# IGLICT/NeRFFaceEditing

Hardware: NVIDIA B200
Metric: rendered rays/sec (48+48 samples) (higher is better)
Workload: dtype f32 (gather, compositing) + bf16x3 split tensor-core MLP with f32 accumulate

## Files before the change

### nerffaceediting_b200/csrc/nfe_field_pipe2.cu

```cuda
#include <type_traits>

#include "nfe_field_launch.cuh"
#include "nfe_mlp_tc.cuh"

namespace nfe {

using namespace tcmlp;

namespace p2 {

constexpr int EPI_GROUPS = 2;
constexpr int MMA_WARP = 8;
constexpr int TAP_WARP0 = 9, TAP_WARPS = 3;
static_assert(TAP_WARPS >= 1 && TAP_WARPS <= 3, "tap warps are warps 9-11");
constexpr int GATHER_WARP0 = 12, GATHER_WARPS = 8;
constexpr int THREADS = (GATHER_WARP0 + GATHER_WARPS) * 32;
constexpr int PASSES_PER_TILE = TILE_M / 4;
constexpr int PER_LONG = (PASSES_PER_TILE + GATHER_WARPS - 1) / GATHER_WARPS;
constexpr int LONG_WARPS = PASSES_PER_TILE - (PER_LONG - 1) * GATHER_WARPS;
static_assert(LONG_WARPS >= 1 && LONG_WARPS <= GATHER_WARPS && PER_LONG >= 2, "bad gather split");
constexpr int TAP_BUFS = 3;
constexpr int GROUP_COLS = 192;
constexpr int P2_TMEM_COLS = 512;
constexpr int COL_D2 = 128;
constexpr int REC_STAGE_STRIDE = 208;

constexpr int REGS_LAUNCH = 65536 / THREADS / 8 * 8;
constexpr int REGS_EPI = 104, REGS_MISC = 64, REGS_GATHER = 104;
static_assert(REGS_EPI > REGS_LAUNCH && REGS_GATHER > REGS_LAUNCH && REGS_MISC < REGS_LAUNCH,
              "the epilogue and gather groups only grow, the MMA / tap group only shrinks");
static_assert(8 * (REGS_EPI - REGS_LAUNCH) + GATHER_WARPS * (REGS_GATHER - REGS_LAUNCH) <= 4 * (REGS_LAUNCH - REGS_MISC),
              "setmaxnreg.inc would wait forever");
static_assert((2 * REGS_EPI + REGS_MISC + (GATHER_WARPS / 4) * REGS_GATHER) * 32 <= 16384, "register file of a sub-partition");

constexpr float LOG2E = 1.4426950408889634f;
constexpr float LN2 = 0.6931471805599453f;

template <int KIND, bool SPLIT>
struct Smem {
    using T = TcTraits<KIND>;
    static constexpr int PARTS = SPLIT ? 2 : 1;
    static constexpr int NETS = T::HAS_B ? 2 : 1;
    alignas(128) unsigned char a1[2][T::SETS][PARTS][A1_BYTES];
    alignas(128) unsigned char b1[NETS][PARTS][B1_BYTES];
    alignas(128) unsigned char b2a[PARTS][(T::N_A / 8) * B2_SBO];
    alignas(128) unsigned char b2b[PARTS][(T::N_B / 8) * B2_SBO];
    alignas(16) uint4 taps[TAP_BUFS][TILE_M][7];
    alignas(16) float aff[TAP_BUFS][2][2][96];
    int aff_item[TAP_BUFS];
    alignas(16) unsigned char recbuf[EPI_GROUPS][TILE_M][REC_STAGE_STRIDE];
    float bias1[NETS][HIDDEN];
    float bias2a[T::N_A];
    float bias2b[T::N_B];
    alignas(8) uint64_t full[2], empty[2];
    uint64_t taps_full[TAP_BUFS], taps_empty[TAP_BUFS];
    uint64_t d1_full[2], a2a_full[2], a2b_full[2], d2a_full[2], d2b_full[2], d2_free[2];
    uint32_t tmem_base;
};

__device__ __forceinline__ void tmem_st8(uint32_t taddr, const uint32_t* r)
{
    asm volatile("tcgen05.st.sync.aligned.32x32b.x8.b32 [%0], {%1, %2, %3, %4, %5, %6, %7, %8};\n"
                 :: "r"(taddr), "r"(r[0]), "r"(r[1]), "r"(r[2]), "r"(r[3]), "r"(r[4]), "r"(r[5]), "r"(r[6]), "r"(r[7]) : "memory");
}

template <int KIND, bool SPLIT>
__device__ void load_params(Smem<KIND, SPLIT>& s, const nfe_mlp& net_a, const nfe_mlp& net_b)
{
    using T = TcTraits<KIND>;
    constexpr int PARTS = SPLIT ? 2 : 1;
    load_weights<PARTS>(s.b1[0][0], B1_BYTES, net_a.w1, net_a.wgain1, HIDDEN, HIDDEN, FEAT, B1_LBO, B1_SBO);
    load_weights<PARTS>(s.b2a[0], sizeof(s.b2a[0]), net_a.w2, net_a.wgain2 * LN2, T::OUT_A, T::N_A, HIDDEN, B2_LBO, B2_SBO);
    for (int i = threadIdx.x; i < HIDDEN; i += blockDim.x) s.bias1[0][i] = folded_bias(net_a.b1, net_a.bgain1, i) * LOG2E;
    for (int i = threadIdx.x; i < T::N_A; i += blockDim.x) s.bias2a[i] = i < T::OUT_A ? folded_bias(net_a.b2, net_a.bgain2, i) : 0.0f;
    if constexpr (T::HAS_B) {
        load_weights<PARTS>(s.b1[1][0], B1_BYTES, net_b.w1, net_b.wgain1, HIDDEN, HIDDEN, FEAT, B1_LBO, B1_SBO);
        load_weights<PARTS>(s.b2b[0], sizeof(s.b2b[0]), net_b.w2, net_b.wgain2 * LN2, T::OUT_B, T::N_B, HIDDEN, B2_LBO, B2_SBO);
        for (int i = threadIdx.x; i < HIDDEN; i += blockDim.x) s.bias1[1][i] = folded_bias(net_b.b1, net_b.bgain1, i) * LOG2E;
        for (int i = threadIdx.x; i < T::N_B; i += blockDim.x) s.bias2b[i] = i < T::OUT_B ? folded_bias(net_b.b2, net_b.bgain2, i) : 0.0f;
    }
}

__device__ __forceinline__ float2 rgb_activation2(float2 x)
{
    const float2 n = fmul2(x, make_float2(-LOG2E, -LOG2E));
    float e0, e1, r0, r1;
    asm("ex2.approx.ftz.f32 %0, %1;" : "=f"(e0) : "f"(n.x));
    asm("ex2.approx.ftz.f32 %0, %1;" : "=f"(e1) : "f"(n.y));
    const float2 d = fadd2(make_float2(e0, e1), make_float2(1.0f, 1.0f));
    asm("rcp.approx.ftz.f32 %0, %1;" : "=f"(r0) : "f"(d.x));
    asm("rcp.approx.ftz.f32 %0, %1;" : "=f"(r1) : "f"(d.y));
    return ffma2(make_float2(r0, r1), make_float2(1.002f, 1.002f), make_float2(-0.001f, -0.001f));
}

template <bool SPLIT>
__device__ __forceinline__ void hidden_in_place(uint32_t taddr, const float* bias1_log2)
{
    const float2 k2 = make_float2(LOG2E, LOG2E), one2 = make_float2(1.0f, 1.0f), neg2 = make_float2(-1.0f, -1.0f);
#pragma unroll 1
    for (int q = 0; q < HIDDEN / 16; ++q) {
        float v[16];
        tc::tmem_ld16(taddr + q * 16, v);
        tc::tmem_ld_wait();
        uint32_t hi[8], lo[8];
#pragma unroll
        for (int i = 0; i < 4; ++i) {
            const float4 b4 = *reinterpret_cast<const float4*>(bias1_log2 + q * 16 + 4 * i);
#pragma unroll
            for (int j = 0; j < 2; ++j) {
                const float2 t = ffma2(make_float2(v[4 * i + 2 * j], v[4 * i + 2 * j + 1]), k2, j ? make_float2(b4.z, b4.w) : make_float2(b4.x, b4.y));
                float e0, e1, l0, l1;
                asm("ex2.approx.ftz.f32 %0, %1;" : "=f"(e0) : "f"(-fabsf(t.x)));
                asm("ex2.approx.ftz.f32 %0, %1;" : "=f"(e1) : "f"(-fabsf(t.y)));
                const float2 s1 = fadd2(make_float2(e0, e1), one2);
                asm("lg2.approx.ftz.f32 %0, %1;" : "=f"(l0) : "f"(s1.x));
                asm("lg2.approx.ftz.f32 %0, %1;" : "=f"(l1) : "f"(s1.y));
                const float2 hh = fadd2(make_float2(fmaxf(t.x, 0.0f), fmaxf(t.y, 0.0f)), make_float2(l0, l1));
                const __nv_bfloat162 p = __floats2bfloat162_rn(hh.x, hh.y);
                hi[2 * i + j] = *reinterpret_cast<const uint32_t*>(&p);
                if (SPLIT) {
                    const float2 d = ffma2(__bfloat1622float2(p), neg2, hh);
                    const __nv_bfloat162 r = __floats2bfloat162_rn(d.x, d.y);
                    lo[2 * i + j] = *reinterpret_cast<const uint32_t*>(&r);
                }
            }
        }
        tmem_st8(taddr + q * 16, hi);
        if (SPLIT) tmem_st8(taddr + q * 16 + 8, lo);
    }
    tc::tmem_st_wait();
}

template <bool SPLIT>
__device__ __forceinline__ void issue_layer2(bool leader, uint32_t tmem_d, uint32_t tmem_h, const unsigned char* b_hi, const unsigned char* b_lo, uint32_t idesc)
{
    uint32_t acc = 0;
    const uint64_t db0 = tc::make_desc(0, B2_LBO, B2_SBO);
    const uint32_t bh = tc::smem_u32(b_hi) >> 4, bl = tc::smem_u32(b_lo) >> 4;
    constexpr int TERMS = SPLIT ? 3 : 1;
#pragma unroll
    for (int t = 0; t < TERMS; ++t) {
        const uint32_t part = (t == 1) ? 8u : 0u;
        const uint32_t b = (t == 2) ? bl : bh;
#pragma unroll
        for (int ks = 0; ks < HIDDEN / 16; ++ks) {
            if (leader) tc::mma_bf16_ts(tmem_d, tmem_h + ks * 16 + part, db0 + (b + ks * ((2 * B2_LBO) >> 4)), idesc, acc);
            acc = 1;
        }
    }
}

struct SampleRef { int64_t idx; int item; int64_t ray; };

__device__ __forceinline__ SampleRef sample_of(const FieldArgs& a, int64_t L, bool small)
{
    SampleRef r;
    r.idx = L;
    if (small) {
        r.item = (int)((uint32_t)L / (uint32_t)a.m);
        r.ray = (int64_t)((uint32_t)L / (uint32_t)a.s_per_ray);
    } else {
        r.item = (int)(L / a.m);
        r.ray = L / a.s_per_ray;
    }
    return r;
}

__device__ __forceinline__ float4 ldg_tap(const float4* lane_base, uint32_t off4, bool streaming)
{
    uint64_t addr;
    asm("mad.wide.u32 %0, %1, 16, %2;" : "=l"(addr) : "r"(off4), "l"(lane_base));
    if (streaming) return __ldcg(reinterpret_cast<const float4*>(addr));
    return __ldg(reinterpret_cast<const float4*>(addr));
}

#ifdef NFE_PIPE_PROFILE
__device__ unsigned long long g_p2_prof[4][16];
#define P2_WAIT(slot, bar, par) do { const long long t0_ = clock64(); tc::mbar_wait(bar, par); prof_[slot] += clock64() - t0_; } while (0)
#else
#define P2_WAIT(slot, bar, par) tc::mbar_wait(bar, par)
#endif

template <int REGS>
__device__ __forceinline__ void regs_inc() { asm volatile("setmaxnreg.inc.sync.aligned.u32 %0;" :: "n"(REGS)); }
template <int REGS>
__device__ __forceinline__ void regs_dec() { asm volatile("setmaxnreg.dec.sync.aligned.u32 %0;" :: "n"(REGS)); }

template <int KIND, bool SPLIT>
__global__ void __launch_bounds__(THREADS, 1) field_pipe2_kernel(FieldArgs a, nfe_mlp net_a, nfe_mlp net_b)
{
    using T = TcTraits<KIND>;
    constexpr int P = SPLIT ? 1 : 0;
    extern __shared__ __align__(128) unsigned char smem_raw[];
    Smem<KIND, SPLIT>& s = *reinterpret_cast<Smem<KIND, SPLIT>*>(smem_raw);
    const int warp = __shfl_sync(0xffffffffu, (int)(threadIdx.x >> 5), 0), lane = threadIdx.x & 31;

    if (warp == MMA_WARP) tc::tmem_alloc(&s.tmem_base, P2_TMEM_COLS);
    if (threadIdx.x == 0) {
        for (int i = 0; i < 2; ++i) {
            tc::mbar_init(&s.full[i], GATHER_WARPS);
            tc::mbar_init(&s.empty[i], 1);
            tc::mbar_init(&s.d1_full[i], 1);
            tc::mbar_init(&s.a2a_full[i], 4);
            tc::mbar_init(&s.a2b_full[i], 4);
            tc::mbar_init(&s.d2a_full[i], 1);
            tc::mbar_init(&s.d2b_full[i], 1);
            tc::mbar_init(&s.d2_free[i], 4);
        }
        for (int i = 0; i < TAP_BUFS; ++i) {
            tc::mbar_init(&s.taps_full[i], TAP_WARPS);
            tc::mbar_init(&s.taps_empty[i], GATHER_WARPS);
        }
        tc::mbar_fence_init();
    }
    load_params(s, net_a, net_b);
    tc::fence_async_smem();
    tc::fence_before_sync();
    __syncthreads();
    tc::fence_after_sync();
    const uint32_t tmem = s.tmem_base;
    const int64_t n_tiles = (a.total + TILE_M - 1) / TILE_M;
    const int64_t G = gridDim.x;
    const int n_my = (int)((n_tiles - blockIdx.x + G - 1) / G);
    const bool skip_b = a.sigma_only && KIND == NFE_DEC_DISENTANGLED;
    const bool has_b = T::HAS_B && !skip_b;
#ifdef NFE_PIPE_PROFILE
    long long prof_[16] = {};
    const long long prof_t0_ = clock64();
#endif

    if (warp >= GATHER_WARP0) {
        const int gw = warp - GATHER_WARP0;
        const int g = lane >> 3, c4 = lane & 7;
        const float4* set_a = reinterpret_cast<const float4*>(a.set_norm) + c4;
        const float4* set_b = reinterpret_cast<const float4*>(a.set_denorm) + c4;
        const bool affine = T::SETS == 2 && a.affine_scale != nullptr;
        const bool rolling = T::SETS == 1 || affine || skip_b;
        const float4* set_r = T::SETS == 2 ? set_a : set_b;
        const int n_pass = gw < LONG_WARPS ? PER_LONG : PER_LONG - 1;
        const int pass0 = gw < LONG_WARPS ? gw * PER_LONG : LONG_WARPS * PER_LONG + (gw - LONG_WARPS) * (PER_LONG - 1);
        const int row0 = 4 * pass0 + g;
        regs_inc<REGS_GATHER>();

        float4 va[12];
        if (n_my > 0) {
            P2_WAIT(0, &s.taps_full[0], 0);
            if (rolling) {
                const uint4* src = s.taps[0][row0];
#pragma unroll
                for (int q = 0; q < 3; ++q) {
                    const uint4 o4 = src[q];
                    va[4 * q] = ldg_tap(set_r, o4.x, q != 0); va[4 * q + 1] = ldg_tap(set_r, o4.y, q != 0);
                    va[4 * q + 2] = ldg_tap(set_r, o4.z, q != 0); va[4 * q + 3] = ldg_tap(set_r, o4.w, q != 0);
                }
            }
        }
        int tb = 0, tb_next = 1;
        for (int it = 0; it < n_my; ++it) {
            const int st = it & 1;
            const bool has_next = it + 1 < n_my;
            P2_WAIT(1, &s.empty[st], ((it >> 1) & 1) ^ 1);
            if (rolling) {
                auto tile_body = [&](auto np_tag) {
                    constexpr int NP = decltype(np_tag)::value;
                    const uint4* tap_row = s.taps[tb][row0];
#pragma unroll 1
                    for (int p = 0; p < NP; ++p) {
                        const int row = row0 + 4 * p;
                        const uint4* cur = tap_row + 4 * p * 7;
                        const bool more = p + 1 < NP;
                        const bool fetch = more || has_next;
                        if (!more && has_next) P2_WAIT(0, &s.taps_full[tb_next], ((it + 1) / TAP_BUFS) & 1);
                        const uint4* nxt = more ? cur + 4 * 7 : s.taps[tb_next][row0];
                        float2 f01[3], f23[3];
#pragma unroll
                        for (int pl = 0; pl < 3; ++pl) {
                            const float4 w4 = *reinterpret_cast<const float4*>(&cur[3 + pl]);
                            const float2 w0 = make_float2(w4.x, w4.x), w1 = make_float2(w4.y, w4.y), w2 = make_float2(w4.z, w4.z), w3 = make_float2(w4.w, w4.w);
                            float2 a01 = fmul2(make_float2(va[4 * pl].x, va[4 * pl].y), w0), a23 = fmul2(make_float2(va[4 * pl].z, va[4 * pl].w), w0);
                            a01 = ffma2(make_float2(va[4 * pl + 1].x, va[4 * pl + 1].y), w1, a01); a23 = ffma2(make_float2(va[4 * pl + 1].z, va[4 * pl + 1].w), w1, a23);
                            a01 = ffma2(make_float2(va[4 * pl + 2].x, va[4 * pl + 2].y), w2, a01); a23 = ffma2(make_float2(va[4 * pl + 2].z, va[4 * pl + 2].w), w2, a23);
                            a01 = ffma2(make_float2(va[4 * pl + 3].x, va[4 * pl + 3].y), w3, a01); a23 = ffma2(make_float2(va[4 * pl + 3].z, va[4 * pl + 3].w), w3, a23);
                            f01[pl] = a01; f23[pl] = a23;
                            if (fetch) {
                                const uint4 o4 = nxt[pl];
                                va[4 * pl] = ldg_tap(set_r, o4.x, pl != 0); va[4 * pl + 1] = ldg_tap(set_r, o4.y, pl != 0);
                                va[4 * pl + 2] = ldg_tap(set_r, o4.z, pl != 0); va[4 * pl + 3] = ldg_tap(set_r, o4.w, pl != 0);
                            }
                        }
                        const float2 third2 = make_float2(1.0f / 3.0f, 1.0f / 3.0f);
                        const float2 fa01 = fmul2(fadd2(fadd2(f01[0], f01[1]), f01[2]), third2), fa23 = fmul2(fadd2(fadd2(f23[0], f23[1]), f23[2]), third2);
                        store_features4<SPLIT>(s.a1[st][0], row, 4 * c4, make_float4(fa01.x, fa01.y, fa23.x, fa23.y));
                        if (affine && !skip_b) {
                            const uint4 meta = cur[6];
                            const float wi[3] = {__uint_as_float(meta.y), __uint_as_float(meta.z), __uint_as_float(meta.w)};
                            const uint32_t rel = a.affine_items == 1 ? 0u : ((uint32_t)((int)meta.x - s.aff_item[tb]) & 1u);
                            const float4* ssc = reinterpret_cast<const float4*>(s.aff[tb][rel][0]) + c4;
                            const float4* ssh = reinterpret_cast<const float4*>(s.aff[tb][rel][1]) + c4;
                            float2 d01[3], d23[3];
#pragma unroll
                            for (int pl = 0; pl < 3; ++pl) {
                                const float4 scl = ssc[pl * 8], shf = ssh[pl * 8];
                                const float2 w2_ = make_float2(wi[pl], wi[pl]);
                                d01[pl] = ffma2(make_float2(scl.x, scl.y), f01[pl], fmul2(make_float2(shf.x, shf.y), w2_));
                                d23[pl] = ffma2(make_float2(scl.z, scl.w), f23[pl], fmul2(make_float2(shf.z, shf.w), w2_));
                            }
                            const float2 fb01 = fmul2(fadd2(fadd2(d01[0], d01[1]), d01[2]), third2), fb23 = fmul2(fadd2(fadd2(d23[0], d23[1]), d23[2]), third2);
                            store_features4<SPLIT>(s.a1[st][T::SETS - 1], row, 4 * c4, make_float4(fb01.x, fb01.y, fb23.x, fb23.y));
                        }
                    }
                };
                if (n_pass == PER_LONG) tile_body(std::integral_constant<int, PER_LONG>{});
                else tile_body(std::integral_constant<int, PER_LONG - 1>{});
            } else {
                if (it > 0) P2_WAIT(0, &s.taps_full[tb], (it / TAP_BUFS) & 1);
#pragma unroll 1
                for (int p = 0; p < n_pass; ++p) {
                    const int row = row0 + 4 * p;
                    TapSet ts;
                    const uint4* src = s.taps[tb][row];
#pragma unroll
                    for (int q = 0; q < 3; ++q) {
                        const uint4 o4 = src[q];
                        ts.off4[4 * q] = (int)o4.x; ts.off4[4 * q + 1] = (int)o4.y; ts.off4[4 * q + 2] = (int)o4.z; ts.off4[4 * q + 3] = (int)o4.w;
                        const uint4 w4 = src[3 + q];
                        ts.w[4 * q] = __uint_as_float(w4.x); ts.w[4 * q + 1] = __uint_as_float(w4.y);
                        ts.w[4 * q + 2] = __uint_as_float(w4.z); ts.w[4 * q + 3] = __uint_as_float(w4.w);
                    }
                    float4 vb[12];
#pragma unroll
                    for (int i = 0; i < 12; ++i) va[i] = ldg_tap(set_a, (uint32_t)ts.off4[i], false);
#pragma unroll
                    for (int i = 0; i < 12; ++i) vb[i] = ldg_tap(set_b, (uint32_t)ts.off4[i], false);
                    store_features4<SPLIT>(s.a1[st][0], row, 4 * c4, gather_reduce(va, ts));
                    store_features4<SPLIT>(s.a1[st][T::SETS - 1], row, 4 * c4, gather_reduce(vb, ts));
                }
            }
            tc::fence_async_smem();
            __syncwarp();
            if (lane == 0) {
                tc::mbar_arrive(&s.full[st]);
                tc::mbar_arrive(&s.taps_empty[tb]);
            }
            tb = tb_next;
            tb_next = tb_next + 1 == TAP_BUFS ? 0 : tb_next + 1;
        }
    } else if (warp >= TAP_WARP0 && warp < TAP_WARP0 + TAP_WARPS) {
        const int tw = warp - TAP_WARP0;
        regs_dec<REGS_MISC>();
        const int64_t set_stride4 = (int64_t)3 * a.H * a.W * (FEAT / 4);
        const bool small = a.total < (1ll << 31);
        struct Raw { float t, o[3], d[3]; int item; bool live; };
        auto owner_of = [&](int it, int h) { return h < TAP_WARPS ? h : (it + h) % TAP_WARPS; };
        auto advance = [&](int& it, int& h) {
            for (;;) {
                if (++h == TILE_M / 32) { h = 0; if (++it >= n_my) return; }
                if (owner_of(it, h) == tw) return;
            }
        };
        auto fetch = [&](int it, int h) {
            Raw r;
            r.t = 0.0f; r.item = 0;
#pragma unroll
            for (int k = 0; k < 3; ++k) r.o[k] = r.d[k] = 0.0f;
            const int64_t L = ((int64_t)blockIdx.x + (int64_t)it * G) * TILE_M + h * 32 + lane;
            r.live = it < n_my && L < a.total;
            if (r.live) {
                const SampleRef sr = sample_of(a, L, small);
                r.item = sr.item;
                if (a.coords) {
                    const float* c = a.coords + sr.idx * 3;
                    r.o[0] = __ldg(c); r.o[1] = __ldg(c + 1); r.o[2] = __ldg(c + 2);
                } else {
                    r.t = __ldg(a.depths + sr.idx);
                    const float* o = a.origins + sr.ray * 3;
                    const float* d = a.dirs + sr.ray * 3;
#pragma unroll
                    for (int k = 0; k < 3; ++k) { r.o[k] = __ldg(o + k); r.d[k] = __ldg(d + k); }
                }
            }
            return r;
        };
        int it = 0, h = -1;
        if (n_my > 0) advance(it, h);
        Raw cur;
        cur.live = false;
        int cit = -1, ch = 0;
#pragma unroll 1
        for (;;) {
            const Raw nxt = fetch(it, h);
            if (cit < 0) {
                if (it >= n_my) break;
                cur = nxt; cit = it; ch = h;
                advance(it, h);
                continue;
            }
            const int tb = cit % TAP_BUFS;
            const bool first = ch == tw;
            if (first) {
                if (cit >= TAP_BUFS) P2_WAIT(2, &s.taps_empty[tb], ((cit / TAP_BUFS) - 1) & 1);
                if (tw == 0 && T::SETS == 2 && a.affine_scale != nullptr) {
                    const int64_t base = ((int64_t)blockIdx.x + (int64_t)cit * G) * TILE_M;
                    const int item0 = a.affine_items == 1 ? 0 : (int)(small ? (uint32_t)base / (uint32_t)a.m : base / a.m);
                    if (lane == 0) s.aff_item[tb] = item0;
                    for (int i = lane; i < 2 * 2 * 24; i += 32) {
                        const int rel = i / 48, which = (i / 24) & 1, c = i % 24;
                        const int item = min(item0 + rel, a.affine_items - 1);
                        const float* src = (which ? a.affine_shift : a.affine_scale) + (int64_t)item * 96;
                        reinterpret_cast<float4*>(s.aff[tb][rel][which])[c] = __ldg(reinterpret_cast<const float4*>(src) + c);
                    }
                }
            }
            {
                const int row = ch * 32 + lane;
                TapSet ts;
#pragma unroll
                for (int i = 0; i < 12; ++i) { ts.off4[i] = 0; ts.w[i] = 0.0f; }
                if (cur.live) {
                    float x, y, z;
                    if (a.coords) { x = cur.o[0]; y = cur.o[1]; z = cur.o[2]; }
                    else { x = ray_point(cur.o[0], cur.t, cur.d[0]); y = ray_point(cur.o[1], cur.t, cur.d[1]); z = ray_point(cur.o[2], cur.t, cur.d[2]); }
                    ts = make_tapset(taps3(__fmul_rn(a.scale, x), __fmul_rn(a.scale, y), __fmul_rn(a.scale, z), a.H, a.W), a.H, a.W);
                    const int item_off = a.plane_batch == 1 ? 0 : (int)(cur.item * set_stride4);
#pragma unroll
                    for (int i = 0; i < 12; ++i) ts.off4[i] += item_off;
                }
                uint4* dst = s.taps[tb][row];
                dst[6] = make_uint4((uint32_t)cur.item, __float_as_uint(((ts.w[0] + ts.w[1]) + ts.w[2]) + ts.w[3]),
                                    __float_as_uint(((ts.w[4] + ts.w[5]) + ts.w[6]) + ts.w[7]), __float_as_uint(((ts.w[8] + ts.w[9]) + ts.w[10]) + ts.w[11]));
#pragma unroll
                for (int q = 0; q < 3; ++q)
                    dst[q] = make_uint4((uint32_t)ts.off4[4 * q], (uint32_t)ts.off4[4 * q + 1], (uint32_t)ts.off4[4 * q + 2], (uint32_t)ts.off4[4 * q + 3]);
#pragma unroll
                for (int q = 0; q < 3; ++q)
                    dst[3 + q] = make_uint4(__float_as_uint(ts.w[4 * q]), __float_as_uint(ts.w[4 * q + 1]), __float_as_uint(ts.w[4 * q + 2]), __float_as_uint(ts.w[4 * q + 3]));
            }
            if (it != cit) {
                __syncwarp();
                if (lane == 0) tc::mbar_arrive(&s.taps_full[tb]);
            }
            if (it >= n_my) break;
            cur = nxt; cit = it; ch = h;
            advance(it, h);
        }
    } else if (warp == MMA_WARP) {
        regs_dec<REGS_MISC>();
        {
            const bool leader = tc::elect_one();
            constexpr uint32_t idesc1 = tc::make_idesc_bf16(TILE_M, HIDDEN);
            constexpr uint32_t idesc2a = tc::make_idesc_bf16(TILE_M, T::N_A);
            constexpr uint32_t idesc2b = tc::make_idesc_bf16(TILE_M, T::N_B);
            auto layer1 = [&](int it) {
                const int st = it & 1;
                const uint32_t tb = tmem + st * GROUP_COLS;
                P2_WAIT(3, &s.full[st], (it >> 1) & 1);
                tc::fence_after_sync();
                issue_gemm<SPLIT>(leader, tb + COL_D1A, s.a1[st][0][0], s.a1[st][0][P], A1_LBO, A1_SBO, s.b1[0][0], s.b1[0][P], B1_LBO, B1_SBO, FEAT, idesc1);
                if (has_b)
                    issue_gemm<SPLIT>(leader, tb + COL_D1B, s.a1[st][T::SETS - 1][0], s.a1[st][T::SETS - 1][P], A1_LBO, A1_SBO, s.b1[T::HAS_B ? 1 : 0][0],
                                      s.b1[T::HAS_B ? 1 : 0][P], B1_LBO, B1_SBO, FEAT, idesc1);
                if (leader) {
                    tc::mma_commit(&s.empty[st]);
                    tc::mma_commit(&s.d1_full[st]);
                }
            };
            if (n_my > 0) layer1(0);
            if (n_my > 1) layer1(1);
            for (int it = 0; it < n_my; ++it) {
                const int gi = it & 1;
                const uint32_t ph = (it >> 1) & 1;
                const uint32_t tb = tmem + gi * GROUP_COLS;
                P2_WAIT(4, &s.a2a_full[gi], ph);
                if (it >= 2) P2_WAIT(5, &s.d2_free[gi], ph ^ 1);
                tc::fence_after_sync();
                issue_layer2<SPLIT>(leader, tb + COL_D2, tb + COL_D1A, s.b2a[0], s.b2a[P], idesc2a);
                if (leader) tc::mma_commit(&s.d2a_full[gi]);
                if (has_b) {
                    P2_WAIT(6, &s.a2b_full[gi], ph);
                    tc::fence_after_sync();
                    issue_layer2<SPLIT>(leader, tb + COL_D2 + T::N_A, tb + COL_D1B, s.b2b[0], s.b2b[P], idesc2b);
                    if (leader) tc::mma_commit(&s.d2b_full[gi]);
                }
                if (it + 2 < n_my) {
                    P2_WAIT(7, has_b ? &s.d2b_full[gi] : &s.d2a_full[gi], ph);
                    layer1(it + 2);
                }
            }
        }
        __syncwarp();
    } else if (warp < MMA_WARP) {
        const int gi = warp >> 2, wq = warp & 3;
        regs_inc<REGS_EPI>();
        const int row = wq * 32 + lane;
        const uint32_t lane_addr = tmem + gi * GROUP_COLS + ((uint32_t)(wq * 32) << 16);
        uint32_t ph = 0;
        for (int it = gi; it < n_my; it += 2, ph ^= 1) {
            const int64_t tile = (int64_t)blockIdx.x + (int64_t)it * G;
            P2_WAIT(8, &s.d1_full[gi], ph);
            tc::fence_after_sync();
#pragma unroll 1
            for (int net = 0; net < (has_b ? 2 : 1); ++net) {
                hidden_in_place<SPLIT>(lane_addr + (net ? COL_D1B : COL_D1A), s.bias1[T::HAS_B ? net : 0]);
                tc::fence_before_sync();
                __syncwarp();
                if (lane == 0) tc::mbar_arrive(net ? &s.a2b_full[gi] : &s.a2a_full[gi]);
            }
            P2_WAIT(9, &s.d2a_full[gi], ph);
            tc::fence_after_sync();
            const int64_t L = tile * TILE_M + row;
            const bool live = L < a.total;
            const int64_t idx = live ? L : 0;
            float4* rec = reinterpret_cast<float4*>(s.recbuf[gi][row]);
            bool done = false;
            if constexpr (KIND == NFE_DEC_DISENTANGLED) {
                {
                    float v[16];
                    tc::tmem_ld16(lane_addr + COL_D2, v);
                    tc::tmem_ld_wait();
#pragma unroll
                    for (int c = 0; c < 4; ++c) {
                        const float4 b4 = *reinterpret_cast<const float4*>(&s.bias2a[4 * c]);
                        const float2 lo2 = fadd2(make_float2(v[4 * c], v[4 * c + 1]), make_float2(b4.x, b4.y));
                        const float2 hi2 = fadd2(make_float2(v[4 * c + 2], v[4 * c + 3]), make_float2(b4.z, b4.w));
                        float4 o = make_float4(lo2.x, lo2.y, hi2.x, hi2.y);
                        if (c == 0) {
                            if (a.density_noise > 0.0f && live) {
                                const uint4 r = philox4x32(a.seed, (uint64_t)idx, a.offset);
                                o.x += normal2(r.x, r.y).x * a.density_noise;
                            }
                            if (live) a.sigma[idx] = o.x;
                        }
                        rec[c] = o;
                    }
                }
                done = a.sigma_only;
                if (!done) {
                    P2_WAIT(10, &s.d2b_full[gi], ph);
                    tc::fence_after_sync();
#pragma unroll 1
                    for (int q = 0; q < T::N_B / 16; ++q) {
                        float v[16];
                        tc::tmem_ld16(lane_addr + COL_D2 + T::N_A + q * 16, v);
                        tc::tmem_ld_wait();
#pragma unroll
                        for (int c = 0; c < 4; ++c) {
                            const float4 b4 = *reinterpret_cast<const float4*>(&s.bias2b[q * 16 + 4 * c]);
                            const float2 lo2 = rgb_activation2(fadd2(make_float2(v[4 * c], v[4 * c + 1]), make_float2(b4.x, b4.y)));
                            const float2 hi2 = rgb_activation2(fadd2(make_float2(v[4 * c + 2], v[4 * c + 3]), make_float2(b4.z, b4.w)));
                            rec[4 + 4 * q + c] = make_float4(lo2.x, lo2.y, hi2.x, hi2.y);
                        }
                    }
                }
            } else {
                float outa[T::N_A];
#pragma unroll
                for (int q = 0; q < T::N_A / 16; ++q) {
                    float v[16];
                    tc::tmem_ld16(lane_addr + COL_D2 + q * 16, v);
                    tc::tmem_ld_wait();
#pragma unroll
                    for (int i = 0; i < 8; ++i) {
                        const float2 o2 = fadd2(make_float2(v[2 * i], v[2 * i + 1]), *reinterpret_cast<const float2*>(&s.bias2a[q * 16 + 2 * i]));
                        outa[q * 16 + 2 * i] = o2.x; outa[q * 16 + 2 * i + 1] = o2.y;
                    }
                }
                float sig = outa[0];
                if (a.density_noise > 0.0f && live) {
                    const uint4 r = philox4x32(a.seed, (uint64_t)idx, a.offset);
                    sig += normal2(r.x, r.y).x * a.density_noise;
                }
                if (live) a.sigma[idx] = sig;
                done = a.sigma_only;
                if (!done) {
                    if (!T::HAS_B) {
                        rec[0] = make_float4(sig, 0.f, 0.f, 0.f);
                        rec[1] = rec[2] = rec[3] = make_float4(0.f, 0.f, 0.f, 0.f);
                    }
#pragma unroll
                    for (int c = 0; c < 8; ++c)
                        rec[4 + c] = make_float4(rgb_activation(outa[1 + 4 * c]), rgb_activation(outa[2 + 4 * c]),
                                                 rgb_activation(outa[3 + 4 * c]), rgb_activation(outa[4 + 4 * c]));
                    if constexpr (T::HAS_B) {
                        P2_WAIT(10, &s.d2b_full[gi], ph);
                        tc::fence_after_sync();
                        float outb[T::N_B];
#pragma unroll
                        for (int q = 0; q < T::N_B / 16; ++q) {
                            float v[16];
                            tc::tmem_ld16(lane_addr + COL_D2 + T::N_A + q * 16, v);
                            tc::tmem_ld_wait();
#pragma unroll
                            for (int i = 0; i < 8; ++i) {
                                const float2 o2 = fadd2(make_float2(v[2 * i], v[2 * i + 1]), *reinterpret_cast<const float2*>(&s.bias2b[q * 16 + 2 * i]));
                                outb[q * 16 + 2 * i] = o2.x; outb[q * 16 + 2 * i + 1] = o2.y;
                            }
                        }
                        rec[0] = make_float4(sig, outb[0], outb[1], outb[2]);
#pragma unroll
                        for (int c = 1; c < 4; ++c) rec[c] = make_float4(outb[4 * c - 1], outb[4 * c], outb[4 * c + 1], outb[4 * c + 2]);
                    }
                }
            }
            tc::fence_before_sync();
            __syncwarp();
            if (lane == 0) tc::mbar_arrive(&s.d2_free[gi]);
            if (!done) {
                const int64_t L0 = tile * TILE_M + wq * 32;
                const int n_rows = (int)min((int64_t)32, a.total - L0);
                const unsigned char* rows = s.recbuf[gi][wq * 32];
                if (a.rec) {
                    float4* gdst = reinterpret_cast<float4*>(a.rec + L0 * 48);
                    int r = lane / 12, c = lane % 12;
#pragma unroll 4
                    for (int k = 0; k < 12; ++k) {
                        const float4 v = *reinterpret_cast<const float4*>(rows + r * REC_STAGE_STRIDE + c * 16);
                        if (r < n_rows) gdst[k * 32 + lane] = v;
                        r += 2; c += 8;
                        if (c >= 12) { c -= 12; r += 1; }
                    }
                } else {
                    float4* gdst = reinterpret_cast<float4*>(a.rgb + L0 * 32);
#pragma unroll 4
                    for (int k = 0; k < 8; ++k) {
                        const int r = 4 * k + (lane >> 3);
                        const float4 v = *reinterpret_cast<const float4*>(rows + r * REC_STAGE_STRIDE + (4 + (lane & 7)) * 16);
                        if (r < n_rows) gdst[k * 32 + lane] = v;
                    }
                    if constexpr (KIND != NFE_DEC_OSG) {
                        float* sdst = a.seg + L0 * 15;
                        int r = lane / 15, c = lane % 15;
#pragma unroll 5
                        for (int k = 0; k < 15; ++k) {
                            const float v = *reinterpret_cast<const float*>(rows + r * REC_STAGE_STRIDE + (1 + c) * 4);
                            if (r < n_rows) sdst[k * 32 + lane] = v;
                            r += 2; c += 2;
                            if (c >= 15) { c -= 15; r += 1; }
                        }
                    }
                }
                __syncwarp();
            }
        }
    } else {
        regs_dec<REGS_MISC>();
    }
#ifdef NFE_PIPE_PROFILE
    if (lane == 0 && !(warp > TAP_WARP0 + TAP_WARPS - 1 && warp < GATHER_WARP0)) {
        const int role = warp >= GATHER_WARP0 ? 0 : (warp >= TAP_WARP0 ? 1 : (warp == MMA_WARP ? 2 : 3));
        prof_[15] = clock64() - prof_t0_;
        for (int i = 0; i < 16; ++i) atomicAdd(&g_p2_prof[role][i], (unsigned long long)prof_[i]);
    }
#endif
    tc::fence_before_sync();
    __syncthreads();
    if (warp == MMA_WARP) tc::tmem_dealloc(tmem, P2_TMEM_COLS);
}

template <int KIND, bool SPLIT>
static int launch_kind(const FieldArgs& a, const nfe_mlp& net_a, const nfe_mlp& net_b, cudaStream_t stream)
{
    const size_t smem = sizeof(Smem<KIND, SPLIT>) + 128;
    static bool configured = false;
    if (!configured) {
        cudaError_t e = cudaFuncSetAttribute(field_pipe2_kernel<KIND, SPLIT>, cudaFuncAttributeMaxDynamicSharedMemorySize, (int)smem);
        if (e != cudaSuccess) { set_error("field_pipe2_kernel: cannot reserve %zu bytes of shared memory: %s", smem, cudaGetErrorString(e)); return 2; }
        configured = true;
    }
    const int64_t n_tiles = (a.total + TILE_M - 1) / TILE_M;
    const int64_t cap = sm_count();
    field_pipe2_kernel<KIND, SPLIT><<<(unsigned)(n_tiles < cap ? n_tiles : cap), THREADS, smem, stream>>>(a, net_a, net_b);
    return check_launch("field_pipe2_kernel");
}

}

int launch_field_pipe2(int kind, int precision, const FieldArgs& a, const nfe_mlp* net_a, const nfe_mlp* net_b, cudaStream_t stream)
{
    if (a.total <= 0) return 0;
    nfe_mlp none = {};
    const bool split = precision == NFE_PREC_BF16X3;
    switch (kind) {
        case NFE_DEC_OSG:
            return split ? p2::launch_kind<NFE_DEC_OSG, true>(a, *net_a, none, stream) : p2::launch_kind<NFE_DEC_OSG, false>(a, *net_a, none, stream);
        case NFE_DEC_DISENTANGLED:
            return split ? p2::launch_kind<NFE_DEC_DISENTANGLED, true>(a, *net_a, *net_b, stream)
                         : p2::launch_kind<NFE_DEC_DISENTANGLED, false>(a, *net_a, *net_b, stream);
        default:
            return split ? p2::launch_kind<NFE_DEC_SEGMENTATION, true>(a, *net_a, *net_b, stream)
                         : p2::launch_kind<NFE_DEC_SEGMENTATION, false>(a, *net_a, *net_b, stream);
    }
}

}

#ifdef NFE_PIPE_PROFILE
NFE_EXPORT int nfe_debug_pipe2_profile(unsigned long long* out64, int reset)
{
    cudaDeviceSynchronize();
    cudaMemcpyFromSymbol(out64, nfe::p2::g_p2_prof, sizeof(unsigned long long) * 64);
    if (reset) { unsigned long long z[64] = {}; cudaMemcpyToSymbol(nfe::p2::g_p2_prof, z, sizeof(z)); }
    return 0;
}
#endif
```

### nerffaceediting_b200/csrc/nfe_mlp_tc.cuh

```cuda
#pragma once
#include "nfe_field.cuh"
#include "nfe_tc.cuh"

namespace nfe { namespace tcmlp {

constexpr int TILE_M = 128;
constexpr int A1_LBO = 160, A1_SBO = 640, A1_BYTES = 16 * A1_SBO;
constexpr int B1_LBO = 128, B1_SBO = 512, B1_BYTES = 8 * B1_SBO;
constexpr int A2_LBO = 128, A2_SBO = 1024, A2_BYTES = 16 * A2_SBO;
constexpr int B2_LBO = 128, B2_SBO = 1024;

template <int KIND> struct TcTraits;
template <> struct TcTraits<NFE_DEC_OSG> { static constexpr int N_A = 48, N_B = 16, OUT_A = 33, OUT_B = 0, SETS = 1; static constexpr bool HAS_B = false; };
template <> struct TcTraits<NFE_DEC_DISENTANGLED> { static constexpr int N_A = 16, N_B = 32, OUT_A = 16, OUT_B = 32, SETS = 2; static constexpr bool HAS_B = true; };
template <> struct TcTraits<NFE_DEC_SEGMENTATION> { static constexpr int N_A = 48, N_B = 16, OUT_A = 33, OUT_B = 15, SETS = 1; static constexpr bool HAS_B = true; };

constexpr int COL_D1A = 0, COL_D1B = 64, COL_D2A = 128, COL_D2B = 176, TMEM_COLS = 256;

template <int KIND, bool SPLIT>
struct Smem {
    using T = TcTraits<KIND>;
    static constexpr int PARTS = SPLIT ? 2 : 1;
    static constexpr int NETS = T::HAS_B ? 2 : 1;
    alignas(128) unsigned char a1[T::SETS][PARTS][A1_BYTES];
    alignas(128) unsigned char b1[NETS][PARTS][B1_BYTES];
    alignas(128) unsigned char a2[NETS][PARTS][A2_BYTES];
    alignas(128) unsigned char b2a[PARTS][(T::N_A / 8) * B2_SBO];
    alignas(128) unsigned char b2b[PARTS][(T::N_B / 8) * B2_SBO];
    float bias1[NETS][HIDDEN];
    float bias2a[T::N_A];
    float bias2b[T::N_B];
    alignas(8) uint64_t bar[2];
    uint32_t tmem_base;
};

__device__ __forceinline__ uint32_t core_offset(int row, int k, int lbo, int sbo)
{
    return (uint32_t)((row >> 3) * sbo + (k >> 3) * lbo + (row & 7) * 16 + (k & 7) * 2);
}

template <int PARTS>
__device__ void load_weights(unsigned char* dst, size_t part_stride, const float* w, float gain, int rows, int rows_pad, int K, int lbo, int sbo)
{
    for (int i = threadIdx.x; i < rows_pad * K; i += blockDim.x) {
        const int n = i / K, k = i % K;
        const float v = n < rows ? __fmul_rn(__ldg(w + n * K + k), gain) : 0.0f;
        __nv_bfloat16 hi, lo;
        tc::split_bf16(v, hi, lo);
        const uint32_t off = core_offset(n, k, lbo, sbo);
        *reinterpret_cast<__nv_bfloat16*>(dst + off) = hi;
        if (PARTS == 2) *reinterpret_cast<__nv_bfloat16*>(dst + part_stride + off) = lo;
    }
}

__device__ __forceinline__ float folded_bias(const float* b, float gain, int i) { return gain != 1.0f ? __fmul_rn(__ldg(b + i), gain) : __ldg(b + i); }

template <int KIND, bool SPLIT>
__device__ void load_params(Smem<KIND, SPLIT>& s, const nfe_mlp& net_a, const nfe_mlp& net_b)
{
    using T = TcTraits<KIND>;
    constexpr int PARTS = SPLIT ? 2 : 1;
    load_weights<PARTS>(s.b1[0][0], B1_BYTES, net_a.w1, net_a.wgain1, HIDDEN, HIDDEN, FEAT, B1_LBO, B1_SBO);
    load_weights<PARTS>(s.b2a[0], sizeof(s.b2a[0]), net_a.w2, net_a.wgain2, T::OUT_A, T::N_A, HIDDEN, B2_LBO, B2_SBO);
    for (int i = threadIdx.x; i < HIDDEN; i += blockDim.x) s.bias1[0][i] = folded_bias(net_a.b1, net_a.bgain1, i);
    for (int i = threadIdx.x; i < T::N_A; i += blockDim.x) s.bias2a[i] = i < T::OUT_A ? folded_bias(net_a.b2, net_a.bgain2, i) : 0.0f;
    if constexpr (T::HAS_B) {
        load_weights<PARTS>(s.b1[1][0], B1_BYTES, net_b.w1, net_b.wgain1, HIDDEN, HIDDEN, FEAT, B1_LBO, B1_SBO);
        load_weights<PARTS>(s.b2b[0], sizeof(s.b2b[0]), net_b.w2, net_b.wgain2, T::OUT_B, T::N_B, HIDDEN, B2_LBO, B2_SBO);
        for (int i = threadIdx.x; i < HIDDEN; i += blockDim.x) s.bias1[1][i] = folded_bias(net_b.b1, net_b.bgain1, i);
        for (int i = threadIdx.x; i < T::N_B; i += blockDim.x) s.bias2b[i] = i < T::OUT_B ? folded_bias(net_b.b2, net_b.bgain2, i) : 0.0f;
    }
}

template <bool SPLIT>
__device__ __forceinline__ void store_features4(unsigned char (*a1)[A1_BYTES], int row, int k0, float4 f)
{
    const __nv_bfloat162 h01 = __floats2bfloat162_rn(f.x, f.y), h23 = __floats2bfloat162_rn(f.z, f.w);
    const uint32_t off = core_offset(row, k0, A1_LBO, A1_SBO);
    *reinterpret_cast<uint2*>(a1[0] + off) = make_uint2(*reinterpret_cast<const uint32_t*>(&h01), *reinterpret_cast<const uint32_t*>(&h23));
    if (SPLIT) {
        const float2 neg2 = make_float2(-1.0f, -1.0f);
        const float2 d01 = ffma2(__bfloat1622float2(h01), neg2, make_float2(f.x, f.y)), d23 = ffma2(__bfloat1622float2(h23), neg2, make_float2(f.z, f.w));
        const __nv_bfloat162 l01 = __floats2bfloat162_rn(d01.x, d01.y), l23 = __floats2bfloat162_rn(d23.x, d23.y);
        *reinterpret_cast<uint2*>(a1[1] + off) = make_uint2(*reinterpret_cast<const uint32_t*>(&l01), *reinterpret_cast<const uint32_t*>(&l23));
    }
}

template <bool SPLIT>
__device__ __forceinline__ void issue_gemm(bool leader, uint32_t tmem_d, const unsigned char* a_hi, const unsigned char* a_lo, int a_lbo, int a_sbo,
                                           const unsigned char* b_hi, const unsigned char* b_lo, int b_lbo, int b_sbo, int K, uint32_t idesc)
{
    const uint64_t da0 = tc::make_desc(0, a_lbo, a_sbo), db0 = tc::make_desc(0, b_lbo, b_sbo);
    const uint32_t ah = tc::smem_u32(a_hi) >> 4, al = tc::smem_u32(a_lo) >> 4, bh = tc::smem_u32(b_hi) >> 4, bl = tc::smem_u32(b_lo) >> 4;
    const uint32_t ak = (uint32_t)(2 * a_lbo) >> 4, bk = (uint32_t)(2 * b_lbo) >> 4;
    uint32_t acc = 0;
    constexpr int TERMS = SPLIT ? 3 : 1;
#pragma unroll
    for (int t = 0; t < TERMS; ++t) {
        const uint32_t a = (t == 1) ? al : ah, b = (t == 2) ? bl : bh;
#pragma unroll 4
        for (int k = 0; k < (K >> 4); ++k) {
            if (leader) tc::mma_bf16_ss(tmem_d, da0 + (a + k * ak), db0 + (b + k * bk), idesc, acc);
            acc = 1;
        }
    }
}
template <bool SPLIT>
__device__ __forceinline__ void issue_gemm(uint32_t tmem_d, const unsigned char* a_hi, const unsigned char* a_lo, int a_lbo, int a_sbo,
                                           const unsigned char* b_hi, const unsigned char* b_lo, int b_lbo, int b_sbo, int K, uint32_t idesc)
{
    issue_gemm<SPLIT>(true, tmem_d, a_hi, a_lo, a_lbo, a_sbo, b_hi, b_lo, b_lbo, b_sbo, K, idesc);
}

template <int KIND, bool SPLIT>
__device__ __forceinline__ void issue_layer1(Smem<KIND, SPLIT>& s, uint32_t tmem)
{
    using T = TcTraits<KIND>;
    constexpr int P = SPLIT ? 1 : 0;
    constexpr uint32_t idesc = tc::make_idesc_bf16(TILE_M, HIDDEN);
    issue_gemm<SPLIT>(tmem + COL_D1A, s.a1[0][0], s.a1[0][P], A1_LBO, A1_SBO, s.b1[0][0], s.b1[0][P], B1_LBO, B1_SBO, FEAT, idesc);
    if constexpr (T::HAS_B) {
        constexpr int SET_B = T::SETS - 1;
        issue_gemm<SPLIT>(tmem + COL_D1B, s.a1[SET_B][0], s.a1[SET_B][P], A1_LBO, A1_SBO, s.b1[1][0], s.b1[1][P], B1_LBO, B1_SBO, FEAT, idesc);
    }
}

template <int KIND, bool SPLIT>
__device__ __forceinline__ void issue_layer2(Smem<KIND, SPLIT>& s, uint32_t tmem)
{
    using T = TcTraits<KIND>;
    constexpr int P = SPLIT ? 1 : 0;
    issue_gemm<SPLIT>(tmem + COL_D2A, s.a2[0][0], s.a2[0][P], A2_LBO, A2_SBO, s.b2a[0], s.b2a[P], B2_LBO, B2_SBO, HIDDEN,
                      tc::make_idesc_bf16(TILE_M, T::N_A));
    if constexpr (T::HAS_B)
        issue_gemm<SPLIT>(tmem + COL_D2B, s.a2[1][0], s.a2[1][P], A2_LBO, A2_SBO, s.b2b[0], s.b2b[P], B2_LBO, B2_SBO, HIDDEN,
                          tc::make_idesc_bf16(TILE_M, T::N_B));
}

template <bool SPLIT>
__device__ __forceinline__ void hidden_epilogue(uint32_t taddr_row, const float* bias1, unsigned char (*a2)[A2_BYTES], int row)
{
#pragma unroll
    for (int q = 0; q < HIDDEN / 16; ++q) {
        float v[16];
        tc::tmem_ld16(taddr_row + q * 16, v);
        tc::tmem_ld_wait();
        uint32_t hi[8], lo[8];
#pragma unroll
        for (int i = 0; i < 8; ++i) {
            const float h0 = softplus_fast(v[2 * i] + bias1[q * 16 + 2 * i]);
            const float h1 = softplus_fast(v[2 * i + 1] + bias1[q * 16 + 2 * i + 1]);
            __nv_bfloat16 a, b, c, d;
            tc::split_bf16(h0, a, c); tc::split_bf16(h1, b, d);
            hi[i] = tc::pack_bf16(a, b); lo[i] = tc::pack_bf16(c, d);
        }
#pragma unroll
        for (int c8 = 0; c8 < 2; ++c8) {
            const uint32_t off = core_offset(row, q * 16 + c8 * 8, A2_LBO, A2_SBO);
            *reinterpret_cast<uint4*>(a2[0] + off) = make_uint4(hi[4 * c8], hi[4 * c8 + 1], hi[4 * c8 + 2], hi[4 * c8 + 3]);
            if (SPLIT) *reinterpret_cast<uint4*>(a2[1] + off) = make_uint4(lo[4 * c8], lo[4 * c8 + 1], lo[4 * c8 + 2], lo[4 * c8 + 3]);
        }
    }
}

template <int KIND, bool SPLIT>
__device__ __forceinline__ void output_epilogue(const Smem<KIND, SPLIT>& s, uint32_t taddr_row, float& sigma, float (&segv)[16], float (&col)[32])
{
    using T = TcTraits<KIND>;
    float a[T::N_A];
#pragma unroll
    for (int q = 0; q < T::N_A / 16; ++q) {
        float v[16];
        tc::tmem_ld16(taddr_row + COL_D2A + q * 16, v);
        tc::tmem_ld_wait();
#pragma unroll
        for (int i = 0; i < 16; ++i) a[q * 16 + i] = v[i] + s.bias2a[q * 16 + i];
    }
    sigma = a[0];
    if constexpr (KIND == NFE_DEC_DISENTANGLED) {
#pragma unroll
        for (int c = 0; c < 15; ++c) segv[c] = a[1 + c];
    } else {
#pragma unroll
        for (int c = 0; c < 32; ++c) col[c] = rgb_activation(a[1 + c]);
    }
    if constexpr (T::HAS_B) {
        float b[T::N_B];
#pragma unroll
        for (int q = 0; q < T::N_B / 16; ++q) {
            float v[16];
            tc::tmem_ld16(taddr_row + COL_D2B + q * 16, v);
            tc::tmem_ld_wait();
#pragma unroll
            for (int i = 0; i < 16; ++i) b[q * 16 + i] = v[i] + s.bias2b[q * 16 + i];
        }
        if constexpr (KIND == NFE_DEC_DISENTANGLED) {
#pragma unroll
            for (int c = 0; c < 32; ++c) col[c] = rgb_activation(b[c]);
        } else {
#pragma unroll
            for (int c = 0; c < 15; ++c) segv[c] = b[c];
        }
    }
}

}}
```

Measured before the change: 33.83 million.

## Gather plane texels with 256-bit loads, 8 channels per lane, plus L2 prefetch

Gather warps now have each lane fetch 8 channels with ld.global.nc.v8.f32 (4 lanes per row, 8 rows per pass) instead of float4 loads with 8 lanes per row. The two-set non-rolling path is folded into a single software-pipelined loop that keeps 6 texels in flight. Tap warps issue prefetch.global.L2 for every tap address ahead of the gather, and features are written to shared memory as 16-byte stores. This cuts load instruction count and L1 transactions in the gather, at the cost of a 32-byte alignment requirement, more register pressure, and extra prefetch instructions in the tap warps.

```diff
diff --git a/nerffaceediting_b200/csrc/nfe_field_pipe2.cu b/nerffaceediting_b200/csrc/nfe_field_pipe2.cu
--- a/nerffaceediting_b200/csrc/nfe_field_pipe2.cu
+++ b/nerffaceediting_b200/csrc/nfe_field_pipe2.cu
@@ -15,10 +15,9 @@
 static_assert(TAP_WARPS >= 1 && TAP_WARPS <= 3, "tap warps are warps 9-11");
 constexpr int GATHER_WARP0 = 12, GATHER_WARPS = 8;
 constexpr int THREADS = (GATHER_WARP0 + GATHER_WARPS) * 32;
-constexpr int PASSES_PER_TILE = TILE_M / 4;
-constexpr int PER_LONG = (PASSES_PER_TILE + GATHER_WARPS - 1) / GATHER_WARPS;
-constexpr int LONG_WARPS = PASSES_PER_TILE - (PER_LONG - 1) * GATHER_WARPS;
-static_assert(LONG_WARPS >= 1 && LONG_WARPS <= GATHER_WARPS && PER_LONG >= 2, "bad gather split");
+constexpr int PASSES_PER_TILE = TILE_M / 8;
+constexpr int PASSES_PER_WARP = PASSES_PER_TILE / GATHER_WARPS;
+static_assert(PASSES_PER_TILE % GATHER_WARPS == 0, "bad gather split");
 constexpr int TAP_BUFS = 3;
 constexpr int GROUP_COLS = 192;
 constexpr int P2_TMEM_COLS = 512;
@@ -166,13 +165,19 @@
     return r;
 }
 
-__device__ __forceinline__ float4 ldg_tap(const float4* lane_base, uint32_t off4, bool streaming)
+__device__ __forceinline__ void ldg_tap8(float* v, const float* set, uint32_t off4, bool streaming)
 {
     uint64_t addr;
-    asm("mad.wide.u32 %0, %1, 16, %2;" : "=l"(addr) : "r"(off4), "l"(lane_base));
-    if (streaming) return __ldcg(reinterpret_cast<const float4*>(addr));
-    return __ldg(reinterpret_cast<const float4*>(addr));
-}
+    asm("mad.wide.u32 %0, %1, 16, %2;" : "=l"(addr) : "r"(off4), "l"(set));
+    if (streaming)
+        asm("ld.global.nc.L1::no_allocate.v8.f32 {%0, %1, %2, %3, %4, %5, %6, %7}, [%8];"
+            : "=f"(v[0]), "=f"(v[1]), "=f"(v[2]), "=f"(v[3]), "=f"(v[4]), "=f"(v[5]), "=f"(v[6]), "=f"(v[7]) : "l"(addr));
+    else
+        asm("ld.global.nc.v8.f32 {%0, %1, %2, %3, %4, %5, %6, %7}, [%8];"
+            : "=f"(v[0]), "=f"(v[1]), "=f"(v[2]), "=f"(v[3]), "=f"(v[4]), "=f"(v[5]), "=f"(v[6]), "=f"(v[7]) : "l"(addr));
+}
+
+__device__ __forceinline__ void l2_prefetch(const float* p) { asm volatile("prefetch.global.L2 [%0];" :: "l"(p)); }
 
 #ifdef NFE_PIPE_PROFILE
 __device__ unsigned long long g_p2_prof[4][16];
@@ -231,111 +236,100 @@
 
     if (warp >= GATHER_WARP0) {
         const int gw = warp - GATHER_WARP0;
-        const int g = lane >> 3, c4 = lane & 7;
-        const float4* set_a = reinterpret_cast<const float4*>(a.set_norm) + c4;
-        const float4* set_b = reinterpret_cast<const float4*>(a.set_denorm) + c4;
+        const int g = lane >> 2, c8 = lane & 3;
+        const uint32_t lane4 = 2 * c8;
         const bool affine = T::SETS == 2 && a.affine_scale != nullptr;
         const bool rolling = T::SETS == 1 || affine || skip_b;
-        const float4* set_r = T::SETS == 2 ? set_a : set_b;
-        const int n_pass = gw < LONG_WARPS ? PER_LONG : PER_LONG - 1;
-        const int pass0 = gw < LONG_WARPS ? gw * PER_LONG : LONG_WARPS * PER_LONG + (gw - LONG_WARPS) * (PER_LONG - 1);
-        const int row0 = 4 * pass0 + g;
+        const bool denorm = affine && !skip_b;
+        const float* set_r = T::SETS == 2 ? a.set_norm : a.set_denorm;
+        const int row0 = 8 * PASSES_PER_WARP * gw + g;
         regs_inc<REGS_GATHER>();
 
-        float4 va[12];
+        float v[6][8];
+        auto load_texel = [&](int i, const uint4* taps_row, const float* set, bool two_sets) {
+            const int pl = i >> 2, k = i & 3;
+            const uint4 o4 = taps_row[pl];
+            const uint32_t off4 = k == 0 ? o4.x : (k == 1 ? o4.y : (k == 2 ? o4.z : o4.w));
+            ldg_tap8(v[i % 6], set, off4 + lane4, !two_sets && pl != 0);
+        };
+        auto mean_step = [](float2 (&acc)[4], const float2 (&f)[4], int pl) {
+            const float2 third2 = make_float2(1.0f / 3.0f, 1.0f / 3.0f);
+#pragma unroll
+            for (int j = 0; j < 4; ++j) {
+                if (pl == 0) acc[j] = f[j];
+                else acc[j] = fadd2(acc[j], f[j]);
+                if (pl == 2) acc[j] = fmul2(acc[j], third2);
+            }
+        };
+        auto tile_runs = [&](auto two_tag, int it, int tb, int tb_next, int st) {
+            constexpr bool TWO = decltype(two_tag)::value;
+            constexpr int RUNS = (TWO ? 2 : 1) * PASSES_PER_WARP;
+            const bool has_next = it + 1 < n_my;
+#pragma unroll 1
+            for (int r = 0; r < RUNS; ++r) {
+                const int set = TWO ? (r & 1) : 0, row = row0 + 8 * (TWO ? r >> 1 : r);
+                const uint4* cur = s.taps[tb][row];
+                const bool more = r + 1 < RUNS;
+                const bool fetch = more || has_next;
+                if (!more && has_next) P2_WAIT(0, &s.taps_full[tb_next], ((it + 1) / TAP_BUFS) & 1);
+                const float* cset = TWO && set ? a.set_denorm : set_r;
+                const float* nset = TWO && !set ? a.set_denorm : set_r;
+                const float* aff = nullptr;
+                if (!TWO && denorm) {
+                    const uint32_t rel = a.affine_items == 1 ? 0u : ((uint32_t)((int)cur[6].x - s.aff_item[tb]) & 1u);
+                    aff = s.aff[tb][rel][0];
+                }
+                float2 fa[4], fb[4];
+#pragma unroll
+                for (int pl = 0; pl < 3; ++pl) {
+                    const float4 w4 = *reinterpret_cast<const float4*>(&cur[3 + pl]);
+                    float2 f[4];
+#pragma unroll
+                    for (int k = 0; k < 4; ++k) {
+                        const int i = 4 * pl + k;
+                        const float wk = k == 0 ? w4.x : (k == 1 ? w4.y : (k == 2 ? w4.z : w4.w));
+                        const float2 w2_ = make_float2(wk, wk);
+#pragma unroll
+                        for (int j = 0; j < 4; ++j) {
+                            const float2 t = make_float2(v[i % 6][2 * j], v[i % 6][2 * j + 1]);
+                            if (k == 0) f[j] = TWO ? ffma2(t, w2_, make_float2(0.0f, 0.0f)) : fmul2(t, w2_);
+                            else f[j] = ffma2(t, w2_, f[j]);
+                        }
+                        if (i + 6 < 12) load_texel(i + 6, cur, cset, TWO);
+                        else if (fetch) load_texel(i - 6, !more ? s.taps[tb_next][row0] : (TWO && !set ? cur : cur + 8 * 7), nset, TWO);
+                    }
+                    mean_step(fa, f, pl);
+                    if (!TWO && denorm) {
+                        const float wi = __uint_as_float(pl == 0 ? cur[6].y : (pl == 1 ? cur[6].z : cur[6].w));
+                        const float2 wi2 = make_float2(wi, wi);
+                        const float4* ssc = reinterpret_cast<const float4*>(aff) + 8 * pl + 2 * c8;
+                        const float4* ssh = ssc + 24;
+                        float2 d[4];
+#pragma unroll
+                        for (int h = 0; h < 2; ++h) {
+                            const float4 scl = ssc[h], shf = ssh[h];
+                            d[2 * h] = ffma2(make_float2(scl.x, scl.y), f[2 * h], fmul2(make_float2(shf.x, shf.y), wi2));
+                            d[2 * h + 1] = ffma2(make_float2(scl.z, scl.w), f[2 * h + 1], fmul2(make_float2(shf.z, shf.w), wi2));
+                        }
+                        mean_step(fb, d, pl);
+                    }
+                }
+                store_features8<SPLIT>(s.a1[st][set ? T::SETS - 1 : 0], row, 8 * c8, fa);
+                if (!TWO && denorm) store_features8<SPLIT>(s.a1[st][T::SETS - 1], row, 8 * c8, fb);
+            }
+        };
+
         if (n_my > 0) {
             P2_WAIT(0, &s.taps_full[0], 0);
-            if (rolling) {
-                const uint4* src = s.taps[0][row0];
-#pragma unroll
-                for (int q = 0; q < 3; ++q) {
-                    const uint4 o4 = src[q];
-                    va[4 * q] = ldg_tap(set_r, o4.x, q != 0); va[4 * q + 1] = ldg_tap(set_r, o4.y, q != 0);
-                    va[4 * q + 2] = ldg_tap(set_r, o4.z, q != 0); va[4 * q + 3] = ldg_tap(set_r, o4.w, q != 0);
-                }
-            }
+#pragma unroll
+            for (int i = 0; i < 6; ++i) load_texel(i, s.taps[0][row0], set_r, !rolling);
         }
         int tb = 0, tb_next = 1;
         for (int it = 0; it < n_my; ++it) {
             const int st = it & 1;
-            const bool has_next = it + 1 < n_my;
             P2_WAIT(1, &s.empty[st], ((it >> 1) & 1) ^ 1);
-            if (rolling) {
-                auto tile_body = [&](auto np_tag) {
-                    constexpr int NP = decltype(np_tag)::value;
-                    const uint4* tap_row = s.taps[tb][row0];
-#pragma unroll 1
-                    for (int p = 0; p < NP; ++p) {
-                        const int row = row0 + 4 * p;
-                        const uint4* cur = tap_row + 4 * p * 7;
-                        const bool more = p + 1 < NP;
-                        const bool fetch = more || has_next;
-                        if (!more && has_next) P2_WAIT(0, &s.taps_full[tb_next], ((it + 1) / TAP_BUFS) & 1);
-                        const uint4* nxt = more ? cur + 4 * 7 : s.taps[tb_next][row0];
-                        float2 f01[3], f23[3];
-#pragma unroll
-                        for (int pl = 0; pl < 3; ++pl) {
-                            const float4 w4 = *reinterpret_cast<const float4*>(&cur[3 + pl]);
-                            const float2 w0 = make_float2(w4.x, w4.x), w1 = make_float2(w4.y, w4.y), w2 = make_float2(w4.z, w4.z), w3 = make_float2(w4.w, w4.w);
-                            float2 a01 = fmul2(make_float2(va[4 * pl].x, va[4 * pl].y), w0), a23 = fmul2(make_float2(va[4 * pl].z, va[4 * pl].w), w0);
-                            a01 = ffma2(make_float2(va[4 * pl + 1].x, va[4 * pl + 1].y), w1, a01); a23 = ffma2(make_float2(va[4 * pl + 1].z, va[4 * pl + 1].w), w1, a23);
-                            a01 = ffma2(make_float2(va[4 * pl + 2].x, va[4 * pl + 2].y), w2, a01); a23 = ffma2(make_float2(va[4 * pl + 2].z, va[4 * pl + 2].w), w2, a23);
-                            a01 = ffma2(make_float2(va[4 * pl + 3].x, va[4 * pl + 3].y), w3, a01); a23 = ffma2(make_float2(va[4 * pl + 3].z, va[4 * pl + 3].w), w3, a23);
-                            f01[pl] = a01; f23[pl] = a23;
-                            if (fetch) {
-                                const uint4 o4 = nxt[pl];
-                                va[4 * pl] = ldg_tap(set_r, o4.x, pl != 0); va[4 * pl + 1] = ldg_tap(set_r, o4.y, pl != 0);
-                                va[4 * pl + 2] = ldg_tap(set_r, o4.z, pl != 0); va[4 * pl + 3] = ldg_tap(set_r, o4.w, pl != 0);
-                            }
-                        }
-                        const float2 third2 = make_float2(1.0f / 3.0f, 1.0f / 3.0f);
-                        const float2 fa01 = fmul2(fadd2(fadd2(f01[0], f01[1]), f01[2]), third2), fa23 = fmul2(fadd2(fadd2(f23[0], f23[1]), f23[2]), third2);
-                        store_features4<SPLIT>(s.a1[st][0], row, 4 * c4, make_float4(fa01.x, fa01.y, fa23.x, fa23.y));
-                        if (affine && !skip_b) {
-                            const uint4 meta = cur[6];
-                            const float wi[3] = {__uint_as_float(meta.y), __uint_as_float(meta.z), __uint_as_float(meta.w)};
-                            const uint32_t rel = a.affine_items == 1 ? 0u : ((uint32_t)((int)meta.x - s.aff_item[tb]) & 1u);
-                            const float4* ssc = reinterpret_cast<const float4*>(s.aff[tb][rel][0]) + c4;
-                            const float4* ssh = reinterpret_cast<const float4*>(s.aff[tb][rel][1]) + c4;
-                            float2 d01[3], d23[3];
-#pragma unroll
-                            for (int pl = 0; pl < 3; ++pl) {
-                                const float4 scl = ssc[pl * 8], shf = ssh[pl * 8];
-                                const float2 w2_ = make_float2(wi[pl], wi[pl]);
-                                d01[pl] = ffma2(make_float2(scl.x, scl.y), f01[pl], fmul2(make_float2(shf.x, shf.y), w2_));
-                                d23[pl] = ffma2(make_float2(scl.z, scl.w), f23[pl], fmul2(make_float2(shf.z, shf.w), w2_));
-                            }
-                            const float2 fb01 = fmul2(fadd2(fadd2(d01[0], d01[1]), d01[2]), third2), fb23 = fmul2(fadd2(fadd2(d23[0], d23[1]), d23[2]), third2);
-                            store_features4<SPLIT>(s.a1[st][T::SETS - 1], row, 4 * c4, make_float4(fb01.x, fb01.y, fb23.x, fb23.y));
-                        }
-                    }
-                };
-                if (n_pass == PER_LONG) tile_body(std::integral_constant<int, PER_LONG>{});
-                else tile_body(std::integral_constant<int, PER_LONG - 1>{});
-            } else {
-                if (it > 0) P2_WAIT(0, &s.taps_full[tb], (it / TAP_BUFS) & 1);
-#pragma unroll 1
-                for (int p = 0; p < n_pass; ++p) {
-                    const int row = row0 + 4 * p;
-                    TapSet ts;
-                    const uint4* src = s.taps[tb][row];
-#pragma unroll
-                    for (int q = 0; q < 3; ++q) {
-                        const uint4 o4 = src[q];
-                        ts.off4[4 * q] = (int)o4.x; ts.off4[4 * q + 1] = (int)o4.y; ts.off4[4 * q + 2] = (int)o4.z; ts.off4[4 * q + 3] = (int)o4.w;
-                        const uint4 w4 = src[3 + q];
-                        ts.w[4 * q] = __uint_as_float(w4.x); ts.w[4 * q + 1] = __uint_as_float(w4.y);
-                        ts.w[4 * q + 2] = __uint_as_float(w4.z); ts.w[4 * q + 3] = __uint_as_float(w4.w);
-                    }
-                    float4 vb[12];
-#pragma unroll
-                    for (int i = 0; i < 12; ++i) va[i] = ldg_tap(set_a, (uint32_t)ts.off4[i], false);
-#pragma unroll
-                    for (int i = 0; i < 12; ++i) vb[i] = ldg_tap(set_b, (uint32_t)ts.off4[i], false);
-                    store_features4<SPLIT>(s.a1[st][0], row, 4 * c4, gather_reduce(va, ts));
-                    store_features4<SPLIT>(s.a1[st][T::SETS - 1], row, 4 * c4, gather_reduce(vb, ts));
-                }
-            }
+            if (rolling) tile_runs(std::false_type{}, it, tb, tb_next, st);
+            else tile_runs(std::true_type{}, it, tb, tb_next, st);
             tc::fence_async_smem();
             __syncwarp();
             if (lane == 0) {
@@ -350,6 +344,8 @@
         regs_dec<REGS_MISC>();
         const int64_t set_stride4 = (int64_t)3 * a.H * a.W * (FEAT / 4);
         const bool small = a.total < (1ll << 31);
+        const float* pf_a = T::SETS == 2 ? a.set_norm : a.set_denorm;
+        const bool pf_both = T::SETS == 2 && a.affine_scale == nullptr && !skip_b;
         struct Raw { float t, o[3], d[3]; int item; bool live; };
         auto owner_of = [&](int it, int h) { return h < TAP_WARPS ? h : (it + h) % TAP_WARPS; };
         auto advance = [&](int& it, int& h) {
@@ -424,6 +420,11 @@
                     const int item_off = a.plane_batch == 1 ? 0 : (int)(cur.item * set_stride4);
 #pragma unroll
                     for (int i = 0; i < 12; ++i) ts.off4[i] += item_off;
+#pragma unroll
+                    for (int i = 0; i < 12; ++i) {
+                        l2_prefetch(pf_a + (uint32_t)ts.off4[i] * 4ull);
+                        if (pf_both) l2_prefetch(a.set_denorm + (uint32_t)ts.off4[i] * 4ull);
+                    }
                 }
                 uint4* dst = s.taps[tb][row];
                 dst[6] = make_uint4((uint32_t)cur.item, __float_as_uint(((ts.w[0] + ts.w[1]) + ts.w[2]) + ts.w[3]),
@@ -677,6 +678,8 @@
 int launch_field_pipe2(int kind, int precision, const FieldArgs& a, const nfe_mlp* net_a, const nfe_mlp* net_b, cudaStream_t stream)
 {
     if (a.total <= 0) return 0;
+    NFE_REQUIRE(((uintptr_t)a.set_norm & 31) == 0 && ((uintptr_t)a.set_denorm & 31) == 0,
+                "field_pipe2_kernel: the channel-last plane sets must be 32-byte aligned (%p, %p)", (const void*)a.set_norm, (const void*)a.set_denorm);
     nfe_mlp none = {};
     const bool split = precision == NFE_PREC_BF16X3;
     switch (kind) {
diff --git a/nerffaceediting_b200/csrc/nfe_mlp_tc.cuh b/nerffaceediting_b200/csrc/nfe_mlp_tc.cuh
--- a/nerffaceediting_b200/csrc/nfe_mlp_tc.cuh
+++ b/nerffaceediting_b200/csrc/nfe_mlp_tc.cuh
@@ -87,6 +87,25 @@
 }
 
 template <bool SPLIT>
+__device__ __forceinline__ void store_features8(unsigned char (*a1)[A1_BYTES], int row, int k0, const float2 (&f)[4])
+{
+    uint32_t hi[4], lo[4];
+#pragma unroll
+    for (int j = 0; j < 4; ++j) {
+        const __nv_bfloat162 h = __floats2bfloat162_rn(f[j].x, f[j].y);
+        hi[j] = *reinterpret_cast<const uint32_t*>(&h);
+        if (SPLIT) {
+            const float2 d = ffma2(__bfloat1622float2(h), make_float2(-1.0f, -1.0f), f[j]);
+            const __nv_bfloat162 l = __floats2bfloat162_rn(d.x, d.y);
+            lo[j] = *reinterpret_cast<const uint32_t*>(&l);
+        }
+    }
+    const uint32_t off = core_offset(row, k0, A1_LBO, A1_SBO);
+    *reinterpret_cast<uint4*>(a1[0] + off) = make_uint4(hi[0], hi[1], hi[2], hi[3]);
+    if (SPLIT) *reinterpret_cast<uint4*>(a1[1] + off) = make_uint4(lo[0], lo[1], lo[2], lo[3]);
+}
+
+template <bool SPLIT>
 __device__ __forceinline__ void issue_gemm(bool leader, uint32_t tmem_d, const unsigned char* a_hi, const unsigned char* a_lo, int a_lbo, int a_sbo,
                                            const unsigned char* b_hi, const unsigned char* b_lo, int b_lbo, int b_sbo, int K, uint32_t idesc)
 {
```

Result: slower. 32.70 million, median of 6 (-3.3%).
